# luuvish/arrow-h264

Hardware: AMD Instinct MI355X
Metric: macroblocks/s (decode reconstruct, post-entropy) 1080p P-frame; % HBM roofline (higher is better)
Workload: dtype u8

## Files before the change

### arrow-h264_amd/csrc/k_recon.hip

```cpp
#include "kernels.h"
#include "mb_inter_sp.h"

using namespace h264r;

#ifndef H264R_INTER_WAVES
#define H264R_INTER_WAVES 4
#endif
struct LdsRegs {
    const uint8_t* plane;
    uint2 refs, hdr;
};
DEV LdsRegs inter4_lds_load(const h264r_batch& b, int pic)
{
    const int t = threadIdx.x;
    const int nsl = min(b.slice_stride, INTER4_LDS_SLICES);
    const h264r_slice* sl = b.slices + (size_t)pic * b.slice_stride;
    LdsRegs r;
    r.plane = b.ref_planes[(size_t)pic * b.ref_planes_stride + min(t, 3 * H264R_MAX_SLOTS - 1)];
    const int ri = min(t, nsl * 4 - 1);
    r.refs = *reinterpret_cast<const uint2*>(&sl[ri >> 2].ref_slot[0][0] + 8 * (ri & 3));
    r.hdr = *reinterpret_cast<const uint2*>(&sl[min(t, nsl - 1)]);
    return r;
}
DEV void inter4_lds_store(const h264r_batch& b, const LdsRegs& r, Inter4Lds& S)
{
    const int t = threadIdx.x;
    const int nsl = min(b.slice_stride, INTER4_LDS_SLICES);
    if (t < 3 * H264R_MAX_SLOTS) S.planes[t] = r.plane;
    if (t < nsl * 4) *reinterpret_cast<uint2*>(&S.ref_slot[t >> 2][0][0] + 8 * (t & 3)) = r.refs;
    if (t < nsl) {
        S.hdr[t] = r.hdr;
        S.slice_type[t] = (uint8_t)(r.hdr.x & 255);
    }
}
DEV void inter4_lds(const h264r_batch& b, int pic, Inter4Lds& S) { inter4_lds_store(b, inter4_lds_load(b, pic), S); }

DEV bool inter4_groups(const Geom& g, int2 rows, int per, int& grp, int& gend)
{
    const int groups = (g.wmb * (rows.y - rows.x) + 15) / 16, gb = (groups + 7) / 8;
    const int band = blockIdx.x & 7;
    grp = band * gb + (blockIdx.x >> 3) * per;
    gend = min(min(grp + per, (band + 1) * gb), groups);
    return grp < gend;
}

extern "C" __global__ __launch_bounds__(256, H264R_INTER_WAVES) void k_inter4r(h264r_batch b, DbInfo* dbinfo, int2 rows,
                                                                               int* sp_flag, uint8_t* recon, int tag,
                                                                               int* zero, int nz, int* zero2, int nz2)
{
    {
        const int nt = (int)(gridDim.x * gridDim.y * blockDim.x);
        const int t = (int)((blockIdx.y * gridDim.x + blockIdx.x) * blockDim.x + threadIdx.x);
        for (int i = t; i < nz; i += nt) zero[i] = 0;
        for (int i = t; i < nz2; i += nt) zero2[i] = 0;
    }
    __shared__ Inter4Lds S;
    __shared__ DbTables T;
    const int pic = blockIdx.y;
    const Geom g = make_geom(b.width_mbs, b.height_mbs);
    int grp, gend;
    if (!inter4_groups(g, rows, H264R_INTER_GROUPS, grp, gend)) return;
    const int lane = threadIdx.x & 63, wave = __builtin_amdgcn_readfirstlane(threadIdx.x >> 6);
    const int aend = rows.y * g.wmb;
    const h264r_slice* slices = b.slices + (size_t)pic * b.slice_stride;
    int a0 = rows.x * g.wmb + (grp * 4 + wave) * 4;
    const uint2 tv = db_tables_load(threadIdx.x);
    Inter4Pre pre = inter4_pre(b, g, pic, a0, aend, lane);
    DbNb nb = dbinfo_pre(b, g, pic, a0, aend, lane);
    const LdsRegs lr = inter4_lds_load(b, pic);
    const int ns = (int)ld_const(&b.pics[pic].num_slices);
    db_tables_store(T, threadIdx.x, tv);
    inter4_lds_store(b, lr, S);
    inter4_plain_mark(S, threadIdx.x, lr.hdr, ns);
    __syncthreads();
    const bool plain = inter4_plain_picture(b, S, ns);
    for (;;) {
        if (a0 >= aend) return;
        bool done = false;
        if ((H264R_INTER_FAST & 2) && plain && inter4_plain_wave(pre, nb, ns)) {
            const uint2 m0 = motion_word<true>(pre.mv[0], pre.ri[0], slices, S, pre.q.slice, 0);
            done = (H264R_INTER_DIAG & 32) ||
                   dbinfo_block<true>(b, pic, inter4_lane(g, a0, aend, lane), S, T, pre.q, m0, inter4_no_list(),
                                      slice_hdr<true>(slices, S, pre.q.slice), nb, dbinfo + (size_t)pic * g.nmb, true);
            if (done) {
                int ln = lane;
                asm volatile("" : "+v"(ln));
                inter4_mbs<true>(b, g, pic, a0, aend, ln, S, sp_flag, pre, recon, tag);
            }
        }
        if (!done) {
            {
                const uint2 m0 = motion_word(pre.mv[0], pre.ri[0], slices, S, pre.q.slice, 0);
                const bool one = (H264R_INTER_FAST & 2) && inter4_one_list(pre, nb);
                uint2 m1 = inter4_no_list();
                if (!one) m1 = motion_word(pre.mv[1], pre.ri[1], slices, S, pre.q.slice, 1);
                if (!(H264R_INTER_DIAG & 32))
                    dbinfo_block(b, pic, inter4_lane(g, a0, aend, lane), S, T, pre.q, m0, m1,
                                 slice_hdr(slices, S, pre.q.slice), nb, dbinfo + (size_t)pic * g.nmb, one);
            }
            int ln = lane;
            asm volatile("" : "+v"(ln));
            inter4_mbs(b, g, pic, a0, aend, ln, S, sp_flag, pre, recon, tag);
        }
        if (++grp >= gend) return;
        a0 = rows.x * g.wmb + (grp * 4 + wave) * 4;
        int ln2 = lane;
        asm volatile("" : "+v"(ln2));
        pre = inter4_pre(b, g, pic, a0, aend, ln2);
        nb = dbinfo_pre(b, g, pic, a0, aend, ln2);
    }
}


extern "C" __global__ __launch_bounds__(256) void k_inter_sp(h264r_batch b, int2 rows, const int* sp_flag, uint8_t* recon,
                                                             int tag)
{
    if (__hip_atomic_load(sp_flag, __ATOMIC_RELAXED, __HIP_MEMORY_SCOPE_AGENT) != tag) return;
    __shared__ Inter4Lds S;
    const Geom g = make_geom(b.width_mbs, b.height_mbs);
    const int lane = threadIdx.x & 63, wave = __builtin_amdgcn_readfirstlane(threadIdx.x >> 6);
    const int groups = (g.wmb * (rows.y - rows.x) + 15) / 16;
    const int aend = rows.y * g.wmb;
    for (int w = blockIdx.x; w < groups * b.num_pics; w += gridDim.x) {
        const int pic = w / groups, grp = w % groups;
        __syncthreads();
        inter4_lds(b, pic, S);
        __syncthreads();
        const int a0 = rows.x * g.wmb + (grp * 4 + wave) * 4;
        if (a0 < aend) inter4_sp_mbs(b, g, pic, a0, aend, lane, S, recon);
    }
}

extern "C" __global__ __launch_bounds__(256) void k_untile(h264r_batch b, int2 rows, const uint8_t* __restrict__ recon)
{
    const Geom g = make_geom(b.width_mbs, b.height_mbs);
    const int pic = blockIdx.y;
    const int t = blockIdx.x * 256 + threadIdx.x, a = rows.x * g.wmb + (t >> 5), k = t & 31;
    if (a >= rows.y * g.wmb) return;
    const int mbx = a % g.wmb, mby = a / g.wmb;
    const uint8_t* mb = recon + ((size_t)pic * g.nmb + a) * RECON_MB;
    if (k < 16) {
        *reinterpret_cast<uint4*>(b.out_y + (size_t)pic * g.ysz + (size_t)(mby * 16 + k) * g.W + mbx * 16) =
            *reinterpret_cast<const uint4*>(mb + k * 16);
    } else {
        const int pl = (k - 16) >> 3, r = k & 7;
        uint8_t* dst = (pl ? b.out_v : b.out_u) + (size_t)pic * g.csz + (size_t)(mby * 8 + r) * g.Wc + mbx * 8;
        *reinterpret_cast<uint2*>(dst) = *reinterpret_cast<const uint2*>(mb + RECON_CB + pl * 64 + r * 8);
    }
}

extern "C" __global__ __launch_bounds__(256) void k_derive444(h264r_batch b, int pl, int qpl, h264r_mb* __restrict__ mbs,
                                                              h264r_slice* __restrict__ slices, h264r_quant* __restrict__ quant,
                                                              const uint8_t** __restrict__ refs, int ntab, int* err)
{
    const int64_t nt = (int64_t)gridDim.x * blockDim.x, t0 = (int64_t)blockIdx.x * blockDim.x + threadIdx.x;
    const int64_t nmb = (int64_t)b.width_mbs * b.height_mbs, P = b.num_pics;
    for (int64_t i = t0; i < P * nmb; i += nt) {
        h264r_mb m = b.mbs[i];
        const int cbpl = m.cbp & 15;
        if (m.mb_type == H264R_I_PCM) m.coef_off += 128u * (uint32_t)pl;
        else m.coef_off += (uint32_t)(pl * (64 * __builtin_popcount(cbpl) + (m.mb_type == H264R_I_16x16 ? 16 : 0)));
        if (pl) { m.qp_y = m.qp_c[pl - 1]; m.qp_scaled[0] = m.qp_scaled[pl]; }
        m.cbp = (uint8_t)cbpl;
        m.chroma_mode = 0;
        mbs[i] = m;
    }
    for (int64_t i = t0; i < P * b.slice_stride; i += nt) {
        h264r_slice x = b.slices[i];
        if (x.slice_type == H264R_SLICE_SP) atomicOr(err, DEV_ERR_FORMAT);
        if (pl) {
            for (int l = 0; l < 2; ++l)
                for (int r = 0; r < H264R_MAX_REFS; ++r) {
                    x.wp_weight[l][r][0] = x.wp_weight[l][r][pl];
                    x.wp_offset[l][r][0] = x.wp_offset[l][r][pl];
                }
            x.luma_log2_wd = x.chroma_log2_wd;
        }
        slices[i] = x;
    }
    constexpr int QW = (int)(sizeof(h264r_quant) / 2);
    constexpr int S4 = 3 * 6 * 16, S8 = 3 * 6 * 64;
    for (int64_t i = t0; i < P * QW; i += nt) {
        const int64_t q = i / QW;
        int k = (int)(i % QW);
        const int16_t* src = reinterpret_cast<const int16_t*>(b.quant + q);
        int from = k;
        if (k < 2 * S4) {
            const int half = k / S4, r = k % S4;
            if (r < 6 * 16) from = half * S4 + qpl * 6 * 16 + r;
        } else {
            const int k8 = k - 2 * S4, half = k8 / S8, r = k8 % S8;
            if (r < 6 * 64) from = 2 * S4 + half * S8 + qpl * 6 * 64 + r;
        }
        reinterpret_cast<int16_t*>(quant + q)[k] = src[from];
    }
    for (int64_t i = t0; i < (int64_t)ntab * 3 * H264R_MAX_SLOTS; i += nt) {
        const int64_t tab = i / (3 * H264R_MAX_SLOTS), e = i % (3 * H264R_MAX_SLOTS), slot = e / 3;
        refs[i] = b.ref_planes[tab * b.ref_planes_stride + 3 * slot + qpl];
    }
    for (int64_t i = t0; i < P; i += nt)
        if (b.pics[i].structure != H264R_FRAME) atomicOr(err, DEV_ERR_NOT_FRAME);
}
```

### arrow-h264_amd/csrc/mb_inter4.h

```cpp
#pragma once
#include "mb_deblock.h"

#ifndef H264R_INTER_DIAG
#define H264R_INTER_DIAG 0
#endif
#ifndef H264R_INTER_FAST
#define H264R_INTER_FAST 3
#endif

namespace h264r {

constexpr int INTER4_MBS = 16;
constexpr int INTER4_LDS_SLICES = 64;
constexpr int INTER4_PLAIN_SLICES = 8;
static_assert(INTER4_PLAIN_SLICES <= INTER4_LDS_SLICES, "a plain picture's slices are all in the LDS copy");

struct Inter4Lds {
    const uint8_t* planes[3 * H264R_MAX_SLOTS];
    uint2 hdr[INTER4_LDS_SLICES];
    int8_t ref_slot[INTER4_LDS_SLICES][2][H264R_MAX_REFS];
    uint8_t slice_type[INTER4_LDS_SLICES];
    uint8_t not_plain[INTER4_PLAIN_SLICES];
};

struct Inter4Lane {
    int blk, bx, by;
    int aa;
    bool valid;
    int mbx, mby;
    int X4, Y4;
    int b8;
    int cb, cr, cc;
    int yoff, coff;
};
DEV Inter4Lane inter4_lane(const Geom& g, int a0, int aend, int lane)
{
    Inter4Lane L;
    const int blk = lane & 15, bx = blk & 3, by = blk >> 2, a = a0 + (lane >> 4);
    L.blk = blk; L.bx = bx; L.by = by;
    L.valid = a < aend;
    L.aa = L.valid ? a : aend - 1;
    L.mbx = L.aa % g.wmb; L.mby = L.aa / g.wmb;
    L.X4 = L.mbx * 4 + bx; L.Y4 = L.mby * 4 + by;
    L.b8 = L.cb = (by >> 1) * 2 + (bx >> 1);
    L.cr = (by & 1) * 2; L.cc = (bx & 1) * 2;
    L.yoff = (by * 4) * 16 + bx * 4;
    L.coff = RECON_CB + (by * 2) * 8 + bx * 2;
    return L;
}

DEV int slice_byte(const h264r_slice* slices, int slice, int off)
{
    const __amdgpu_buffer_rsrc_t rs = __builtin_amdgcn_make_buffer_rsrc(const_cast<h264r_slice*>(slices + slice), 0,
                                                                        (int)sizeof(h264r_slice), 0x00020000);
    return __builtin_amdgcn_raw_buffer_load_b8(rs, off, 0, 0);
}
template <bool NEAR = false>
DEV int slice_type_of(const h264r_slice* slices, const Inter4Lds& S, int slice)
{
    int t = S.slice_type[min(slice, INTER4_LDS_SLICES - 1)];
    if constexpr (!NEAR)
        if (slice >= INTER4_LDS_SLICES) t = slice_byte(slices, slice, (int)offsetof(h264r_slice, slice_type));
    return t;
}

template <bool NEAR = false>
DEV uint2 slice_hdr(const h264r_slice* slices, const Inter4Lds& S, int slice)
{
    if (NEAR || slice < INTER4_LDS_SLICES) return S.hdr[NEAR ? min(slice, INTER4_LDS_SLICES - 1) : slice];
    return *reinterpret_cast<const uint2*>(&slices[slice]);
}

template <bool NEAR = false>
DEV uint2 motion_word(uint32_t mv, int ri, const h264r_slice* slices, const Inter4Lds& S, int slice, int l)
{
    const bool has = ri >= 0 && ri < H264R_MAX_REFS;
    const int ric = has ? ri : 0;
    int slot = S.ref_slot[min(slice, INTER4_LDS_SLICES - 1)][l][ric];
    if constexpr (!NEAR)
        if (slice >= INTER4_LDS_SLICES)
            slot = (int8_t)slice_byte(slices, slice, (int)offsetof(h264r_slice, ref_slot) + l * H264R_MAX_REFS + ric);
    slot = has ? slot : -1;
    return make_uint2(mv, (uint32_t)(uint8_t)ri | ((uint32_t)(uint8_t)slot << 8));
}
DEV uint2 block_motion(const h264r_batch& b, const h264r_slice* slices, const Inter4Lds& S, size_t at, int slice, int l)
{
    return motion_word(b.mv[at], b.ref_idx[at], slices, S, slice, l);
}

DEV h264r_mb mb_lane(const h264r_mb* p)
{
    const uint4* q = reinterpret_cast<const uint4*>(p);
    const uint4 w0 = q[0], w1 = q[1];
    h264r_mb m;
    uint32_t* w = reinterpret_cast<uint32_t*>(&m);
    w[0] = w0.x; w[1] = w0.y; w[2] = w0.z; w[3] = w0.w; w[4] = w1.x; w[5] = w1.y; w[6] = w1.z; w[7] = w1.w;
    return m;
}

struct Inter4Pre {
    h264r_mb q;
    uint32_t mv[2];
    int ri[2];
};
DEV Inter4Pre inter4_pre(const h264r_batch& b, const Geom& g, int pic, int a0, int aend, int lane)
{
    const Inter4Lane L = inter4_lane(g, a0, aend, lane);
    const int mi = L.Y4 * g.W4 + L.X4;
    const size_t mbase = (size_t)pic * 2 * g.motion_plane;
    Inter4Pre p;
    p.q = mb_lane(&b.mbs[(size_t)pic * g.nmb + L.aa]);
#pragma unroll
    for (int l = 0; l < 2; ++l) {
        p.mv[l] = b.mv[mbase + l * g.motion_plane + mi];
        p.ri[l] = b.ref_idx[mbase + l * g.motion_plane + mi];
    }
    return p;
}

struct DbNb {
    h264r_mb L, U;
    uint32_t lmv[2], umv[2];
    int lri[2], uri[2];
};
DEV DbNb dbinfo_pre(const h264r_batch& b, const Geom& g, int pic, int a0, int aend, int lane)
{
    const Inter4Lane L = inter4_lane(g, a0, aend, lane);
    const int aa = L.aa, mi = L.Y4 * g.W4 + L.X4;
    const int li = L.X4 > 0 ? mi - 1 : mi, ui = L.Y4 > 0 ? mi - g.W4 : mi;
    const size_t mbase = (size_t)pic * 2 * g.motion_plane;
    const h264r_mb* mbs = b.mbs + (size_t)pic * g.nmb;
    DbNb n;
    n.L = mb_lane(&mbs[L.mbx > 0 ? aa - 1 : aa]);
    n.U = mb_lane(&mbs[L.mby > 0 ? aa - g.wmb : aa]);
#pragma unroll
    for (int l = 0; l < 2; ++l) {
        n.lmv[l] = b.mv[mbase + l * g.motion_plane + li];
        n.lri[l] = b.ref_idx[mbase + l * g.motion_plane + li];
        n.umv[l] = b.mv[mbase + l * g.motion_plane + ui];
        n.uri[l] = b.ref_idx[mbase + l * g.motion_plane + ui];
    }
    return n;
}

DEV int sel16(uint32_t lo, uint32_t hi, int c) { return (int16_t)(((c & 2) ? hi : lo) >> (16 * (c & 1))); }

typedef short s16x2 __attribute__((ext_vector_type(2)));
typedef float f32x2 __attribute__((ext_vector_type(2)));
DEV s16x2 as_s16x2(uint32_t v) { return __builtin_bit_cast(s16x2, v); }
DEV uint32_t as_u32(s16x2 v) { return __builtin_bit_cast(uint32_t, v); }
DEV s16x2 splat16(short v) { return (s16x2){v, v}; }
DEV s16x2 pk_max(s16x2 a, s16x2 b) { return __builtin_elementwise_max(a, b); }
DEV s16x2 pk_min(s16x2 a, s16x2 b) { return __builtin_elementwise_min(a, b); }
DEV s16x2 pk_clip255(s16x2 a) { return pk_min(pk_max(a, splat16(0)), splat16(255)); }
DEV s16x2 pk_lo(uint32_t a, uint32_t b) { return as_s16x2(__builtin_amdgcn_perm(b, a, 0x05040100u)); }
DEV s16x2 pk_hi(uint32_t a, uint32_t b) { return as_s16x2(__builtin_amdgcn_perm(b, a, 0x07060302u)); }
DEV s16x2 pk_sat(int a, int b) { return __builtin_bit_cast(s16x2, __builtin_amdgcn_cvt_pk_i16(a, b)); }
DEV void idct4_pk(s16x2& a, s16x2& b, s16x2& c, s16x2& d)
{
    const s16x2 e0 = a + c, e1 = a - c, e2 = (b >> splat16(1)) - d, e3 = b + (d >> splat16(1));
    a = e0 + e3; b = e1 + e2; c = e1 - e2; d = e0 - e3;
}
constexpr uint32_t DQ4_BIAS = 1u << 27;
DEV uint32_t dq4_biased(int lev, int scale, int per) { return ((uint32_t)(lev * scale) * (1u << per) + 0x80000008u) >> 4; }
DEV uint32_t abs_acc_biased(uint32_t u, uint32_t acc)
{
    uint32_t r;
    asm("v_sad_u32 %0, %1, %2, %3" : "=v"(r) : "v"(u), "s"(DQ4_BIAS), "v"(acc));
    return r;
}
constexpr uint32_t PK_RES_MAX = 32700;
DEV uint32_t construct4(uint32_t pred, s16x2 r01, s16x2 r23)
{
    const s16x2 p01 = as_s16x2(__builtin_amdgcn_perm(0, pred, 0x0c010c00u)), p23 = as_s16x2(__builtin_amdgcn_perm(0, pred, 0x0c030c02u));
    const s16x2 s01 = pk_clip255(__builtin_elementwise_add_sat(p01, r01)), s23 = pk_clip255(__builtin_elementwise_add_sat(p23, r23));
    return __builtin_amdgcn_perm(as_u32(s23), as_u32(s01), 0x06040200u);
// ... 239 lines not shown
    const bool noref = !mb_is_intra(pre.q) && pre.ri[0] < 0;
    return inter4_one_list(pre, nb) && !__any(far || noref);
}

template <bool ONE>
DEV void dbinfo_records(const h264r_mb& q, const h264r_mb& L, const h264r_mb& U, const MotionRef& mq, const MotionRef& ml,
                        const MotionRef& mu, int blk, int hasL, int hasU, uint32_t qsh0, int l_type, int u_type, int fld,
                        const DbTables& T, DbInfo* __restrict__ out)
{
    const int bx = blk & 3, by = blk >> 2;
    const int q_type = qsh0 & 255, idc = (qsh0 >> 8) & 255;
    const int offa = (int8_t)((qsh0 >> 16) & 255), offb = (int8_t)(qsh0 >> 24);
    const int mvlim = fld ? 2 : 4;
    const int q_intra = mb_is_intra(q);
    const int fl = idc == 0 ? hasL : (idc == 2 && hasL && L.slice == q.slice);
    const int ft = idc == 0 ? hasU : (idc == 2 && hasU && U.slice == q.slice);
    const int t8 = (q.flags & H264R_MBF_T8x8) != 0;
    const int pskip = q_type == H264R_SLICE_P && q.mb_type == H264R_P_SKIP;
    const int special_q = special_slice(q_type);
#pragma unroll
    for (int hor = 0; hor < 2; ++hor) {
        const int e = hor ? by : bx, s = hor ? bx : by;
        const int en = idc != 1 && (e == 0 ? (hor ? ft : fl) : ((e & 1) ? !t8 : 1));
        int v = 0;
        if (en) {
            const int p_flags = e == 0 ? (hor ? U.flags : L.flags) : q.flags;
            const int p_cbp = e == 0 ? (hor ? U.cbp_blks : L.cbp_blks) : q.cbp_blks;
            const int special = special_q || (e == 0 && special_slice(hor ? u_type : l_type));
            const int intra = q_intra || (p_flags & H264R_MBF_INTRA) != 0;
            const int blkQ = 4 * by + bx;
            const int blkP = hor ? (e == 0 ? 12 + bx : blkQ - 4) : (e == 0 ? blkQ + 3 : blkQ - 1);
            const int coded = ((q.cbp_blks >> blkQ) & 1) || ((p_cbp >> blkP) & 1);
            const int same_part = e > 0 && (q.mb_type == H264R_P_16x16 ||
                                            q.mb_type == (hor ? H264R_P_8x16 : H264R_P_16x8));
            if (!hor) {
                if (special) v = e == 0 ? 4 : 3;
                else if (e > 0 && pskip) v = 0;
                else if (e == 0 && intra) v = 4;
                else if (intra) v = 3;
                else if (coded) v = 2;
                else if (same_part) v = 0;
                else v = ONE ? bs_compare_one(mq, ml, mvlim) : bs_compare(mq, ml, mvlim);
            } else {
                if (e == 0 && !fld && (special || intra)) v = 4;
                else if (special || intra) v = 3;
                else if (e > 0 && pskip) v = 0;
                else if (coded) v = 2;
                else if (same_part) v = 0;
                else v = ONE ? bs_compare_one(mq, mu, mvlim) : bs_compare(mq, mu, mvlim);
            }
        }
        out->bs[hor * 16 + e * 4 + s] = (uint8_t)v;
    }
    if (blk < 9) {
        const int pl = blk / 3, which = blk - pl * 3;
        const h264r_mb& P = which == 0 ? L : (which == 1 ? U : q);
        const int qp = mb_qp(P, pl), qq = mb_qp(q, pl);
        out->par[blk] = edge_word(qp, qq, offa, offb, T.ab, T.tc0);
    }
}

template <bool PLAIN = false>
DEV bool dbinfo_block(const h264r_batch& b, int pic, const Inter4Lane& ln, const Inter4Lds& S, const DbTables& T,
                      const h264r_mb& q, uint2 m0, uint2 m1, uint2 qsh, const DbNb& nb, DbInfo* __restrict__ dbout, bool one)
{
    const int bx = ln.bx, by = ln.by;
    const h264r_slice* slices = b.slices + (size_t)pic * b.slice_stride;
    const int hasL = ln.mbx > 0, hasU = ln.mby > 0;
    const h264r_mb& L = nb.L;
    const h264r_mb& U = nb.U;
    const int lsl = bx > 0 ? q.slice : L.slice, usl = by > 0 ? q.slice : U.slice;
    const uint2 l0 = motion_word<PLAIN>(nb.lmv[0], nb.lri[0], slices, S, lsl, 0);
    const uint2 u0 = motion_word<PLAIN>(nb.umv[0], nb.uri[0], slices, S, usl, 0);
    uint2 l1 = inter4_no_list(), u1 = l1;
    if constexpr (!PLAIN) {
        if (!one) {
            l1 = motion_word(nb.lmv[1], nb.lri[1], slices, S, lsl, 1);
            u1 = motion_word(nb.umv[1], nb.uri[1], slices, S, usl, 1);
        }
    }
    const int l_type = slice_type_of<PLAIN>(slices, S, L.slice), u_type = slice_type_of<PLAIN>(slices, S, U.slice);
    const int fld = (int)__builtin_amdgcn_readfirstlane(ld_const(&b.pics[pic].structure)) != H264R_FRAME;
    const MotionRef mq = motion_of(m0, m1), ml = motion_of(l0, l1), mu = motion_of(u0, u1);
    const bool both_missing = !mb_is_intra(q) && mq.ref[0] < 0 && (ml.ref[0] < 0 || mu.ref[0] < 0);
    if constexpr (PLAIN) {
        if (__any(ln.valid && both_missing)) return false;
    }
    if (ln.valid) {
        DbInfo* out = dbout + ln.aa;
        if constexpr (PLAIN) {
            dbinfo_records<true>(q, L, U, mq, ml, mu, ln.blk, hasL, hasU, qsh.x, l_type, u_type, fld, T, out);
        } else {
            if (one) one = !__any(both_missing);
            if (one) dbinfo_records<true>(q, L, U, mq, ml, mu, ln.blk, hasL, hasU, qsh.x, l_type, u_type, fld, T, out);
            else dbinfo_records<false>(q, L, U, mq, ml, mu, ln.blk, hasL, hasU, qsh.x, l_type, u_type, fld, T, out);
        }
    }
    return true;
}

DEV void inter4_pcm(uint8_t* rmb, const Inter4Lane& L, const int16_t* lv)
{
    const uint8_t* raw = reinterpret_cast<const uint8_t*>(lv);
#pragma unroll
    for (int r = 0; r < 4; ++r)
        *reinterpret_cast<uint32_t*>(rmb + L.yoff + r * 16) = *reinterpret_cast<const uint32_t*>(raw + (L.by * 4 + r) * 16 + L.bx * 4);
#pragma unroll
    for (int pl = 0; pl < 2; ++pl)
#pragma unroll
        for (int r = 0; r < 2; ++r)
            *reinterpret_cast<uint16_t*>(rmb + L.coff + pl * 64 + r * 8) =
                *reinterpret_cast<const uint16_t*>(raw + 256 + pl * 64 + (L.by * 2 + r) * 8 + L.bx * 2);
}

DEV void inter4_mc(const Geom& g, const Inter4Lane& L, const Inter4Lds& S, int structure, int fld, uint2 mw, int rr, bool use,
                   uint32_t (&tY)[4], uint32_t (&tC)[2])
{
    tY[0] = tY[1] = tY[2] = tY[3] = 0x80808080u;
    tC[0] = tC[1] = 0x80808080u;
    const int ref = (int8_t)((mw.y >> 8) & 255);
    const int slot = ref & 31, bot = fld & (ref >> 6);
    const bool ok = use && ref >= 0 && (ref & ~H264R_REF_BOTTOM) < H264R_MAX_SLOTS && rr < H264R_MAX_REFS &&
                    S.planes[slot * 3];
    const int mvx = (int16_t)(mw.x & 0xFFFF), mvy = (int16_t)(mw.x >> 16);
    const int vx = L.X4 * 16 + mvx, vy = L.Y4 * 16 + mvy;
    const int x = vx >> 2, y = vy >> 2;
    {
        uint32_t w[9][3];
        if constexpr (H264R_INTER_DIAG & 4) {
            tY[0] = tY[1] = tY[2] = tY[3] = (uint32_t)(vx ^ vy);
        } else {
            if (ok) luma_window_global(S.planes[slot * 3] + bot * g.W, g.W, g.W << fld, g.H, x, y, w);
            if constexpr (H264R_INTER_DIAG & 2) {
                if (ok) {
                    uint32_t acc = 0;
#pragma unroll
                    for (int r = 0; r < 9; ++r) acc ^= w[r][0] ^ w[r][1] ^ w[r][2];
                    tY[0] = tY[1] = tY[2] = tY[3] = acc;
                }
            } else {
                if (ok) luma_block_pred(w, g.W, x, vx & 3, vy & 3, tY);
            }
        }
    }
    const int vyc = vy + (fld && bot != (structure == H264R_BOTTOM_FIELD) ? (bot ? -2 : 2) : 0);
    if constexpr (H264R_INTER_DIAG & 8) {
        tC[0] = tC[1] = (uint32_t)vyc;
    } else {
        if (ok) chroma_block_pred2(S.planes[slot * 3 + 1] + bot * g.Wc, S.planes[slot * 3 + 2] + bot * g.Wc, g.Wc,
                                   g.Wc << fld, g.Hc, vx >> 3, vyc >> 3, vx & 7, vyc & 7, tC);
    }
}

template <bool PLAIN = false>
DEV void inter4_predict(const h264r_batch& b, const Geom& g, int pic, const Inter4Lane& L, const Inter4Lds& S,
                        const h264r_slice* __restrict__ qs, int wp_mode, uint2 m0, uint2 m1, uint32_t (&predY)[4],
                        uint32_t (&predC)[2])
{
    const int structure = (int)__builtin_amdgcn_readfirstlane(ld_const(&b.pics[pic].structure));
    const int fld = structure != H264R_FRAME;
    const int r0 = (int8_t)(m0.y & 255);
    if constexpr (PLAIN) {
        inter4_mc(g, L, S, structure, fld, m0, r0, true, predY, predC);
        return;
    }
    const int r1 = (int8_t)(m1.y & 255);
    const int dir = (r0 >= 0 && r1 >= 0) ? 2 : (r0 >= 0 ? 0 : 1);
    uint32_t pY[2][4] = {{0, 0, 0, 0}, {0, 0, 0, 0}}, pC[2][2] = {{0, 0}, {0, 0}};
#pragma unroll 1
    for (int l = 0; l < 2; ++l) {
        const uint2 mw = l ? m1 : m0;
        const int rr = l ? r1 : r0;
        const bool use = rr >= 0;
        if (!__any(use)) continue;
        uint32_t tY[4], tC[2];
        inter4_mc(g, L, S, structure, fld, mw, rr, use, tY, tC);
        const bool l1 = l != 0;
#pragma unroll
        for (int i = 0; i < 4; ++i) {
            pY[0][i] = (use && !l1) ? tY[i] : pY[0][i];
            pY[1][i] = (use && l1) ? tY[i] : pY[1][i];
        }
#pragma unroll
        for (int k = 0; k < 2; ++k) {
            pC[0][k] = (use && !l1) ? tC[k] : pC[0][k];
            pC[1][k] = (use && l1) ? tC[k] : pC[1][k];
        }
    }
    WpPar wpp[3] = {};
    if (wp_mode != 0) {
        const WpRaw wr = wp_raw(qs, r0, r1);
#pragma unroll
        for (int pl = 0; pl < 3; ++pl) wpp[pl] = wp_params(wr, wp_mode, dir, pl);
    }
#pragma unroll
    for (int i = 0; i < 4; ++i) predY[i] = wp_combine4(wpp[0], wp_mode, dir, pY[0][i], pY[1][i]);
#pragma unroll
    for (int pl = 0; pl < 2; ++pl) predC[pl] = wp_combine4(wpp[1 + pl], wp_mode, dir, pC[0][pl], pC[1][pl]);
}

struct Inter4Res {
    uint4 lev[2], lsc[2];
    uint32_t clev[2][2], csc[2][2];
    uint2 cdc[2];
    int cdcs[2];
};
DEV Inter4Res inter4_res_load(const h264r_mb& q, const Inter4Lane& L, const int16_t* lv, const h264r_quant* __restrict__ qt)
{
    Inter4Res R = {};
    const int cbpc = q.cbp >> 4, qpl = q.qp_scaled[0];
    const int by = L.by, bx = L.bx;
    const int loff = b8_offset(q.cbp, L.b8);
    if (loff >= 0) {
        if (!(q.flags & H264R_MBF_T8x8)) {
            const uint4* p = reinterpret_cast<const uint4*>(lv + loff + ((by & 1) * 2 + (bx & 1)) * 16);
            R.lev[0] = p[0]; R.lev[1] = p[1];
            const uint4* s = reinterpret_cast<const uint4*>(&qt->scale4x4[1][0][qpl % 6][0]);
            R.lsc[0] = s[0]; R.lsc[1] = s[1];
        } else {
            const int16_t* p = lv + loff + (by & 1) * 32 + (bx & 1) * 4;
            const int16_t* s = &qt->scale8x8[1][0][qpl % 6][(by & 1) * 32 + (bx & 1) * 4];
            const uint2 r0 = ld8(p), r1 = ld8(p + 8), r2 = ld8(p + 16), r3 = ld8(p + 24);
            R.lev[0] = make_uint4(r0.x, r0.y, r1.x, r1.y); R.lev[1] = make_uint4(r2.x, r2.y, r3.x, r3.y);
            const uint2 s0 = ld8(s), s1 = ld8(s + 8), s2 = ld8(s + 16), s3 = ld8(s + 24);
            R.lsc[0] = make_uint4(s0.x, s0.y, s1.x, s1.y); R.lsc[1] = make_uint4(s2.x, s2.y, s3.x, s3.y);
        }
    }
    if (cbpc) {
        const LevelOffs lo = level_offsets(q);
#pragma unroll
        for (int pl = 0; pl < 2; ++pl) {
            const int qpc = q.qp_scaled[1 + pl];
            R.cdc[pl] = ld8(lv + lo.cdc + pl * 4);
            R.cdcs[pl] = qt->scale4x4[1][1 + pl][qpc % 6][0];
            if (cbpc == 2) {
#pragma unroll
                for (int r = 0; r < 2; ++r) {
                    R.clev[pl][r] = *reinterpret_cast<const uint32_t*>(lv + lo.cac + pl * 64 + L.cb * 16 + (L.cr + r) * 4 + L.cc);
                    R.csc[pl][r] = *reinterpret_cast<const uint32_t*>(&qt->scale4x4[1][1 + pl][qpc % 6][(L.cr + r) * 4 + L.cc]);
                }
            }
        }
    }
    return R;
}
DEV int res_at(const uint4 (&w)[2], int i, int c) { return sel16((i & 1) ? w[i >> 1].z : w[i >> 1].x, (i & 1) ? w[i >> 1].w : w[i >> 1].y, c); }
DEV int level_at(const Inter4Res& R, int i, int c) { return res_at(R.lev, i, c); }
DEV int scale_at(const Inter4Res& R, int i, int c) { return res_at(R.lsc, i, c); }
DEV void luma_dequant(const Inter4Res& R, int per, int t8, int (&d)[4][4])
{
    const int drnd = t8 ? 32 : 8, dsh = t8 ? 6 : 4;
#pragma unroll
    for (int i = 0; i < 4; ++i)
#pragma unroll
        for (int c = 0; c < 4; ++c) d[i][c] = ((level_at(R, i, c) * scale_at(R, i, c)) * (1 << per) + drnd) >> dsh;
}
DEV void pack_res(const int (&res)[4][4], s16x2 (&rp)[4][2])
{
#pragma unroll
    for (int i = 0; i < 4; ++i) {
        rp[i][0] = pk_sat(res[i][0], res[i][1]);
        rp[i][1] = pk_sat(res[i][2], res[i][3]);
    }
}

DEV void luma_res_bypass(const h264r_mb& q, const Inter4Lane& L, const Inter4Res& R, int t8, s16x2 (&rp)[4][2])
{
    const int bx = L.bx, by = L.by;
    int d[4][4];
#pragma unroll
    for (int i = 0; i < 4; ++i)
#pragma unroll
        for (int c = 0; c < 4; ++c) d[i][c] = level_at(R, i, c);
    const uint32_t* qw = reinterpret_cast<const uint32_t*>(&q);
    const uint64_t ipw = (uint64_t)qw[5] | ((uint64_t)qw[6] << 32);
    const int bk = t8 ? L.b8 : (by >> 1) * 8 + (bx >> 1) * 4 + (by & 1) * 2 + (bx & 1);
    const int mode = (int)((ipw >> (4 * bk)) & 15);
    const bool vert = mode == 0, horz = mode == 1;
#pragma unroll
    for (int i = 1; i < 4; ++i)
#pragma unroll
        for (int c = 0; c < 4; ++c) d[i][c] += vert ? d[i - 1][c] : 0;
#pragma unroll
    for (int c = 1; c < 4; ++c)
#pragma unroll
        for (int i = 0; i < 4; ++i) d[i][c] += horz ? d[i][c - 1] : 0;
#pragma unroll
    for (int c = 0; c < 4; ++c) {
        const int up = lane_xor4(d[3][c]);
#pragma unroll
        for (int i = 0; i < 4; ++i) d[i][c] += (t8 && vert && (by & 1)) ? up : 0;
    }
#pragma unroll
    for (int i = 0; i < 4; ++i) {
        const int left = lane_xor1(d[i][3]);
#pragma unroll
        for (int c = 0; c < 4; ++c) d[i][c] += (t8 && horz && (bx & 1)) ? left : 0;
    }
    pack_res(d, rp);
}

template <bool PK>
DEV void luma_res_4x4(const Inter4Res& R, int per, int t8, s16x2 (&rp)[4][2])
{
    bool pk = PK;
    uint32_t u[4][4];
    if (pk) {
        uint32_t gs = 0;
#pragma unroll
        for (int i = 0; i < 4; ++i)
#pragma unroll
            for (int c = 0; c < 4; ++c) {
                u[i][c] = dq4_biased(level_at(R, i, c), scale_at(R, i, c), per);
                gs = abs_acc_biased(u[i][c], gs);
            }
        pk = !__any(gs > PK_RES_MAX);
    }
    if (pk) {
        s16x2 A[4], B[4];
#pragma unroll
        for (int c = 0; c < 4; ++c) {
            A[c] = pk_lo(u[0][c], u[1][c]);
            B[c] = pk_lo(u[2][c], u[3][c]);
        }
        A[0] += (s16x2){32, 0};
        idct4_pk(A[0], A[1], A[2], A[3]);
        idct4_pk(B[0], B[1], B[2], B[3]);
#pragma unroll
        for (int h = 0; h < 2; ++h) {
            s16x2 x0 = pk_lo(as_u32(A[2 * h]), as_u32(A[2 * h + 1])), x1 = pk_hi(as_u32(A[2 * h]), as_u32(A[2 * h + 1]));
            s16x2 x2 = pk_lo(as_u32(B[2 * h]), as_u32(B[2 * h + 1])), x3 = pk_hi(as_u32(B[2 * h]), as_u32(B[2 * h + 1]));
            idct4_pk(x0, x1, x2, x3);
            rp[0][h] = x0 >> splat16(6); rp[1][h] = x1 >> splat16(6);
            rp[2][h] = x2 >> splat16(6); rp[3][h] = x3 >> splat16(6);
        }
    } else {
        int d[4][4], res[4][4];
        if constexpr (PK) {
#pragma unroll
            for (int i = 0; i < 4; ++i)
#pragma unroll
                for (int c = 0; c < 4; ++c) d[i][c] = (int)(u[i][c] - DQ4_BIAS);
        } else {
            luma_dequant(R, per, t8, d);
        }
        idct4x4_inplace(d);
#pragma unroll
        for (int i = 0; i < 4; ++i)
#pragma unroll
            for (int c = 0; c < 4; ++c) res[i][c] = (d[i][c] + 32) >> 6;
        pack_res(res, rp);
    }
}

DEV void luma_res_8x8(const Inter4Lane& L, const Inter4Res& R, int per, int t8, s16x2 (&rp)[4][2])
{
    const int bx = L.bx, by = L.by;
    int d[4][4], e4[4][4], res[4][4];
    luma_dequant(R, per, t8, d);
#pragma unroll
    for (int i = 0; i < 4; ++i) {
        int in[8], outv[8];
#pragma unroll
        for (int c = 0; c < 4; ++c) {
            const int ov = lane_xor1(d[i][c]);
            in[c] = (bx & 1) ? ov : d[i][c];
            in[4 + c] = (bx & 1) ? d[i][c] : ov;
        }
        idct8(in, outv);
        const int mx = -(bx & 1);
#pragma unroll
        for (int c = 0; c < 4; ++c) e4[i][c] = (outv[c] & ~mx) | (outv[4 + c] & mx);
    }
#pragma unroll
    for (int c = 0; c < 4; ++c) {
        int in[8], outv[8];
#pragma unroll
        for (int i = 0; i < 4; ++i) {
            in[i] = lane_lo4(e4[i][c]);
            in[4 + i] = lane_hi4(e4[i][c]);
        }
        idct8(in, outv);
        const int my = -(by & 1);
#pragma unroll
        for (int i = 0; i < 4; ++i) res[i][c] = t8 ? ((outv[i] & ~my) | (outv[4 + i] & my)) : 0;
    }
    if (!t8) idct4x4_inplace(d);
#pragma unroll
    for (int i = 0; i < 4; ++i)
#pragma unroll
        for (int c = 0; c < 4; ++c) res[i][c] = ((t8 ? res[i][c] : d[i][c]) + 32) >> 6;
    pack_res(res, rp);
}

template <bool PK>
DEV void inter4_luma_residual(const h264r_mb& q, const Inter4Lane& L, const Inter4Res& R, s16x2 (&rp)[4][2])
{
#pragma unroll
    for (int i = 0; i < 4; ++i) rp[i][0] = rp[i][1] = splat16(0);
    if (!__any((q.cbp & 15) != 0)) return;
    const int t8 = (q.flags & H264R_MBF_T8x8) != 0, per = q.qp_scaled[0] / 6;
    if (q.flags & H264R_MBF_BYPASS) luma_res_bypass(q, L, R, t8, rp);
    else if (!__any(t8 != 0)) luma_res_4x4<PK>(R, per, t8, rp);
    else luma_res_8x8(L, R, per, t8, rp);
}
DEV void luma_res_stub(const Inter4Res& R, s16x2 (&rp)[4][2])
{
#pragma unroll
    for (int i = 0; i < 4; ++i) rp[i][0] = rp[i][1] = splat16(0);
    rp[0][0].x = (short)((R.lev[0].x ^ R.lev[0].y ^ R.lev[0].z ^ R.lev[0].w ^ R.lev[1].x ^ R.lev[1].y ^ R.lev[1].z ^ R.lev[1].w ^
                          R.lsc[0].x ^ R.lsc[1].y) & 3);
}

DEV void inter4_store_luma(uint8_t* rmb, const Inter4Lane& L, const uint32_t (&predY)[4], const s16x2 (&rp)[4][2])
{
#pragma unroll
    for (int i = 0; i < 4; ++i) *reinterpret_cast<uint32_t*>(rmb + L.yoff + i * 16) = construct4(predY[i], rp[i][0], rp[i][1]);
}
DEV void inter4_store_luma_16b(uint8_t* rmb, const Inter4Lane& L, const uint32_t (&predY)[4], const s16x2 (&rp)[4][2])
{
    uint32_t wv4[4];
#pragma unroll
    for (int i = 0; i < 4; ++i) wv4[i] = construct4(predY[i], rp[i][0], rp[i][1]);
    *reinterpret_cast<uint4*>(rmb + L.blk * 16) = make_uint4(wv4[0], wv4[1], wv4[2], wv4[3]);
}

DEV s16x2 lane_xor1(s16x2 v) { return as_s16x2((uint32_t)lane_xor1((int)as_u32(v))); }
DEV s16x2 lane_lo4(s16x2 v) { return as_s16x2((uint32_t)lane_lo4((int)as_u32(v))); }
DEV s16x2 lane_hi4(s16x2 v) { return as_s16x2((uint32_t)lane_hi4((int)as_u32(v))); }
template <auto Op, typename T>
DEV void quad_rows(T& a, T& b, int cc)
{
    const T o0 = lane_xor1(a), o1 = lane_xor1(b);
    T d0 = cc ? o0 : a, d1 = cc ? o1 : b, d2 = cc ? a : o0, d3 = cc ? b : o1;
    Op(d0, d1, d2, d3);
    a = cc ? d2 : d0;
    b = cc ? d3 : d1;
}
template <auto Op, bool XOR4 = false, typename T>
DEV void quad_cols(T& a, T& b, int cr)
{
    T d0, d1, d2, d3;
    if constexpr (XOR4) {
        const T o0 = lane_xor4(a), o1 = lane_xor4(b);
        d0 = cr ? o0 : a; d1 = cr ? o1 : b; d2 = cr ? a : o0; d3 = cr ? b : o1;
    } else {
        d0 = lane_lo4(a); d1 = lane_lo4(b); d2 = lane_hi4(a); d3 = lane_hi4(b);
    }
    Op(d0, d1, d2, d3);
    a = cr ? d2 : d0;
    b = cr ? d3 : d1;
}

template <bool PK>
DEV void inter4_chroma_residual(const h264r_mb& q, const Inter4Lane& L, const Inter4Res& R, s16x2 (&rcp)[2][2])
{
    const int cb = L.cb, cr = L.cr, cc = L.cc;
    const int cbpc = q.cbp >> 4;
    const bool byp = (q.flags & H264R_MBF_BYPASS) != 0;
#pragma unroll
    for (int pl = 0; pl < 2; ++pl) rcp[pl][0] = rcp[pl][1] = splat16(0);
    if (!__any(cbpc != 0)) return;
    const bool dcl_lane = cr == 0 && cc == 0;
    uint32_t k[2][2][2];
    int dcl[2];
#pragma unroll
    for (int pl = 0; pl < 2; ++pl) {
        const int qpc = q.qp_scaled[1 + pl], per = qpc / 6;
#pragma unroll
        for (int r = 0; r < 2; ++r)
#pragma unroll
            for (int c = 0; c < 2; ++c)
                k[pl][r][c] = dq4_biased((int16_t)(R.clev[pl][r] >> (16 * c)), (int16_t)(R.csc[pl][r] >> (16 * c)), per);
        const int c00 = (int16_t)(R.cdc[pl].x & 0xFFFF), c01 = (int16_t)(R.cdc[pl].x >> 16);
        const int c10 = (int16_t)(R.cdc[pl].y & 0xFFFF), c11 = (int16_t)(R.cdc[pl].y >> 16);
        const int e00 = c00 + c01, e01 = c00 - c01, e10 = c10 + c11, e11 = c10 - c11;
        const int ea = (cb & 1) ? e01 : e00, eb = (cb & 1) ? e11 : e10;
        const int f = ea + (eb ^ -(cb >> 1)) + (cb >> 1);
        if (dcl_lane) k[pl][0][0] = (uint32_t)(cbpc ? ((f * R.cdcs[pl]) * (1 << per)) >> 5 : 0) + DQ4_BIAS;
        dcl[pl] = cb == 0 ? c00 : cb == 1 ? c01 : cb == 2 ? c10 : c11;
    }
    bool pk = PK;
    if (pk) {
        uint32_t gs[2];
#pragma unroll
        for (int pl = 0; pl < 2; ++pl)
            gs[pl] = abs_acc_biased(k[pl][0][0], abs_acc_biased(k[pl][0][1], abs_acc_biased(k[pl][1][0], abs_acc_biased(k[pl][1][1], 0))));
        int m = byp ? 0 : (int)max(gs[0], gs[1]);
        int o = lane_xor1(m);
        asm volatile("" : "+v"(o));
        m = (int)((uint32_t)m + (uint32_t)o);
        int lo = lane_lo4(m), hi = lane_hi4(m);
        asm volatile("" : "+v"(lo), "+v"(hi));
        pk = !__any((uint32_t)lo + (uint32_t)hi > PK_RES_MAX);
    }
    if (pk) {
        s16x2 K[2][2];
#pragma unroll
        for (int r = 0; r < 2; ++r)
#pragma unroll
            for (int c = 0; c < 2; ++c) K[r][c] = pk_lo(k[0][r][c], k[1][r][c]);
        K[0][0] += splat16(dcl_lane ? 32 : 0);
#pragma unroll
        for (int r = 0; r < 2; ++r) quad_rows<idct4_pk>(K[r][0], K[r][1], cc);
#pragma unroll
        for (int c = 0; c < 2; ++c) quad_cols<idct4_pk>(K[0][c], K[1][c], cr);
#pragma unroll
        for (int r = 0; r < 2; ++r) {
            const uint32_t r0 = as_u32(K[r][0] >> splat16(6)), r1 = as_u32(K[r][1] >> splat16(6));
            rcp[0][r] = pk_lo(r0, r1);
            rcp[1][r] = pk_hi(r0, r1);
        }
    } else {
#pragma unroll
        for (int pl = 0; pl < 2; ++pl) {
            int t[2][2];
#pragma unroll
            for (int r = 0; r < 2; ++r) {
                t[r][0] = (int)(k[pl][r][0] - DQ4_BIAS);
                t[r][1] = (int)(k[pl][r][1] - DQ4_BIAS);
                quad_rows<idct4_inplace>(t[r][0], t[r][1], cc);
            }
#pragma unroll
            for (int c = 0; c < 2; ++c) quad_cols<idct4_inplace>(t[0][c], t[1][c], cr);
#pragma unroll
            for (int r = 0; r < 2; ++r) rcp[pl][r] = pk_sat((t[r][0] + 32) >> 6, (t[r][1] + 32) >> 6);
        }
    }
    if (byp) {
#pragma unroll
        for (int pl = 0; pl < 2; ++pl) {
            rcp[pl][0] = dcl_lane ? pk_hi((uint32_t)dcl[pl] << 16, R.clev[pl][0]) : as_s16x2(R.clev[pl][0]);
            rcp[pl][1] = as_s16x2(R.clev[pl][1]);
        }
    }
}
DEV void chroma_res_stub(const Inter4Res& R, s16x2 (&rcp)[2][2])
{
#pragma unroll
    for (int pl = 0; pl < 2; ++pl) {
        rcp[pl][0] = rcp[pl][1] = splat16(0);
        rcp[pl][0].x = (short)((R.clev[pl][0] ^ R.clev[pl][1] ^ R.csc[pl][0] ^ R.csc[pl][1] ^ R.cdc[pl].x ^ R.cdc[pl].y ^ (uint32_t)R.cdcs[pl]) & 3);
    }
}

DEV void inter4_store_chroma(uint8_t* rmb, const Inter4Lane& L, const uint32_t (&predC)[2], const s16x2 (&rcp)[2][2])
{
#pragma unroll
    for (int pl = 0; pl < 2; ++pl) {
        uint8_t* cdst = rmb + L.coff + pl * 64;
#pragma unroll
        for (int r = 0; r < 2; ++r) {
            const s16x2 pr = as_s16x2(__builtin_amdgcn_perm(0, predC[pl], r ? 0x0c030c02u : 0x0c010c00u));
            const s16x2 sv = pk_clip255(__builtin_elementwise_add_sat(pr, rcp[pl][r]));
            *reinterpret_cast<uint16_t*>(cdst + r * 8) = (uint16_t)__builtin_amdgcn_perm(0, as_u32(sv), 0x0c0c0200u);
        }
    }
}

template <bool PLAIN = false>
DEV void inter4_mbs(const h264r_batch& b, const Geom& g, int pic, int a0, int aend, int lane,
                    const Inter4Lds& S, int* sp_flag, const Inter4Pre& pre, uint8_t* __restrict__ recon, int tag)
{
    constexpr int DIAG = H264R_INTER_DIAG;
    constexpr bool PK = (H264R_INTER_FAST & 1) != 0;
    const Inter4Lane L = inter4_lane(g, a0, aend, lane);
    const h264r_slice* slices = b.slices + (size_t)pic * b.slice_stride;
    const h264r_mb q = pre.q;
    const uint2 qsh = slice_hdr<PLAIN>(slices, S, q.slice);
    const uint2 m0 = motion_word<PLAIN>(pre.mv[0], pre.ri[0], slices, S, q.slice, 0);
    uint2 m1 = inter4_no_list();
    if constexpr (!PLAIN) m1 = motion_word(pre.mv[1], pre.ri[1], slices, S, q.slice, 1);

    const bool pcm = q.mb_type == H264R_I_PCM;
    if (!L.valid || (mb_is_intra(q) && !pcm)) return;
    if constexpr (!PLAIN)
        if ((qsh.x & 255) == H264R_SLICE_SP && !mb_is_intra(q)) { *sp_flag = tag; return; }
    if (pcm) { inter4_pcm(recon_mb(recon, g, pic, L.aa), L, b.levels + q.coef_off); return; }

    uint32_t predY[4], predC[2];
    inter4_predict<PLAIN>(b, g, pic, L, S, &slices[q.slice], qsh.y & 255, m0, m1, predY, predC);
    Inter4Res R = {};
    if constexpr (!(DIAG & 16)) R = inter4_res_load(q, L, b.levels + q.coef_off, &b.quant[pic]);
    uint8_t* const rmb = recon_mb(recon, g, pic, L.aa);

    s16x2 rp[4][2];
    if constexpr (DIAG & (16 | 64)) luma_res_stub(R, rp);
    else inter4_luma_residual<PK>(q, L, R, rp);
    if constexpr (DIAG & 1) inter4_store_luma_16b(rmb, L, predY, rp);
    else inter4_store_luma(rmb, L, predY, rp);

    s16x2 rcp[2][2];
    if constexpr (DIAG & (16 | 128)) chroma_res_stub(R, rcp);
    else inter4_chroma_residual<PK>(q, L, R, rcp);
    inter4_store_chroma(rmb, L, predC, rcp);
}

}
```

Before: 745.3 million.

## Park live prediction and MB state in LDS to raise wave occupancy

Adds a per-thread LDS parking area where the non-plain inter path spills prediction words, list-1 motion, and selected macroblock record fields across the residual decode, then reloads them. It also raises the occupancy target in launch bounds from 4 to 5 waves. The bypass residual now reads its intra-mode dwords straight from global memory instead of keeping them live. The aim is lower VGPR pressure so more waves fit per SIMD. The cost is about 18KB of extra LDS per block plus extra LDS traffic, and the LDS growth may itself cap occupancy.

```diff
diff --git a/arrow-h264_amd/csrc/k_recon.hip b/arrow-h264_amd/csrc/k_recon.hip
--- a/arrow-h264_amd/csrc/k_recon.hip
+++ b/arrow-h264_amd/csrc/k_recon.hip
@@ -4,7 +4,7 @@
 using namespace h264r;
 
 #ifndef H264R_INTER_WAVES
-#define H264R_INTER_WAVES 4
+#define H264R_INTER_WAVES 5
 #endif
 struct LdsRegs {
     const uint8_t* plane;
@@ -56,6 +56,7 @@
     }
     __shared__ Inter4Lds S;
     __shared__ DbTables T;
+    __shared__ Inter4Park P;
     const int pic = blockIdx.y;
     const Geom g = make_geom(b.width_mbs, b.height_mbs);
     int grp, gend;
@@ -78,14 +79,16 @@
         if (a0 >= aend) return;
         bool done = false;
         if ((H264R_INTER_FAST & 2) && plain && inter4_plain_wave(pre, nb, ns)) {
-            const uint2 m0 = motion_word<true>(pre.mv[0], pre.ri[0], slices, S, pre.q.slice, 0);
+            uint2 m0 = motion_word<true>(pre.mv[0], pre.ri[0], slices, S, pre.q.slice, 0);
+            asm volatile("" : "+v"(m0.y));
             done = (H264R_INTER_DIAG & 32) ||
                    dbinfo_block<true>(b, pic, inter4_lane(g, a0, aend, lane), S, T, pre.q, m0, inter4_no_list(),
                                       slice_hdr<true>(slices, S, pre.q.slice), nb, dbinfo + (size_t)pic * g.nmb, true);
             if (done) {
                 int ln = lane;
-                asm volatile("" : "+v"(ln));
-                inter4_mbs<true>(b, g, pic, a0, aend, ln, S, sp_flag, pre, recon, tag);
+                uint2 mm = m0;
+                asm volatile("" : "+v"(ln), "+v"(mm.x), "+v"(mm.y));
+                inter4_mbs<true>(b, g, pic, a0, aend, ln, S, sp_flag, pre, recon, tag, nullptr, mm);
             }
         }
         if (!done) {
@@ -100,7 +103,7 @@
             }
             int ln = lane;
             asm volatile("" : "+v"(ln));
-            inter4_mbs(b, g, pic, a0, aend, ln, S, sp_flag, pre, recon, tag);
+            inter4_mbs(b, g, pic, a0, aend, ln, S, sp_flag, pre, recon, tag, &P);
         }
         if (++grp >= gend) return;
         a0 = rows.x * g.wmb + (grp * 4 + wave) * 4;
diff --git a/arrow-h264_amd/csrc/mb_inter4.h b/arrow-h264_amd/csrc/mb_inter4.h
--- a/arrow-h264_amd/csrc/mb_inter4.h
+++ b/arrow-h264_amd/csrc/mb_inter4.h
@@ -22,6 +22,34 @@
     uint8_t slice_type[INTER4_LDS_SLICES];
     uint8_t not_plain[INTER4_PLAIN_SLICES];
 };
+
+constexpr int PARK_PRED = 0;
+constexpr int PARK_M1 = 12;
+constexpr int PARK_Q = 14;
+constexpr int INTER4_PARK_SLOTS = 18;
+struct Inter4Park {
+    uint32_t w[INTER4_PARK_SLOTS][256];
+};
+typedef __attribute__((address_space(3))) volatile uint32_t lds_vdword;
+DEV void park_put(Inter4Park& P, int slot, uint32_t v) { *(lds_vdword*)&P.w[slot][threadIdx.x] = v; }
+DEV uint32_t park_get(Inter4Park& P, int slot) { return *(lds_vdword*)&P.w[slot][threadIdx.x]; }
+constexpr int PARK_Q_N = 4;
+constexpr int PARK_Q_WORD[PARK_Q_N] = {0, 3, 2, 4};
+DEV void park_put_mb(Inter4Park& P, const h264r_mb& q)
+{
+    const uint32_t* w = reinterpret_cast<const uint32_t*>(&q);
+#pragma unroll
+    for (int k = 0; k < PARK_Q_N; ++k) park_put(P, PARK_Q + k, w[PARK_Q_WORD[k]]);
+}
+template <int FIRST = PARK_Q_N>
+DEV h264r_mb park_get_mb(Inter4Park& P)
+{
+    h264r_mb q = {};
+    uint32_t* w = reinterpret_cast<uint32_t*>(&q);
+#pragma unroll
+    for (int k = 0; k < FIRST; ++k) w[PARK_Q_WORD[k]] = park_get(P, PARK_Q + k);
+    return q;
+}
 
 struct Inter4Lane {
     int blk, bx, by;
@@ -567,10 +595,10 @@
     }
 }
 
-template <bool PLAIN = false>
+template <bool PLAIN = false, bool PARK = false>
 DEV void inter4_predict(const h264r_batch& b, const Geom& g, int pic, const Inter4Lane& L, const Inter4Lds& S,
                         const h264r_slice* __restrict__ qs, int wp_mode, uint2 m0, uint2 m1, uint32_t (&predY)[4],
-                        uint32_t (&predC)[2])
+                        uint32_t (&predC)[2], Inter4Park* park = nullptr)
 {
     const int structure = (int)__builtin_amdgcn_readfirstlane(ld_const(&b.pics[pic].structure));
     const int fld = structure != H264R_FRAME;
@@ -581,29 +609,56 @@
     }
     const int r1 = (int8_t)(m1.y & 255);
     const int dir = (r0 >= 0 && r1 >= 0) ? 2 : (r0 >= 0 ? 0 : 1);
+    if constexpr (PARK) {
+        park_put(*park, PARK_M1, m1.x);
+        park_put(*park, PARK_M1 + 1, m1.y);
+    }
     uint32_t pY[2][4] = {{0, 0, 0, 0}, {0, 0, 0, 0}}, pC[2][2] = {{0, 0}, {0, 0}};
+    bool parked[2] = {false, false};
 #pragma unroll 1
     for (int l = 0; l < 2; ++l) {
-        const uint2 mw = l ? m1 : m0;
         const int rr = l ? r1 : r0;
         const bool use = rr >= 0;
         if (!__any(use)) continue;
+        uint2 mw = l ? m1 : m0;
+        if constexpr (PARK)
+            if (l) mw = make_uint2(park_get(*park, PARK_M1), park_get(*park, PARK_M1 + 1));
         uint32_t tY[4], tC[2];
         inter4_mc(g, L, S, structure, fld, mw, rr, use, tY, tC);
         const bool l1 = l != 0;
-#pragma unroll
-        for (int i = 0; i < 4; ++i) {
-            pY[0][i] = (use && !l1) ? tY[i] : pY[0][i];
-            pY[1][i] = (use && l1) ? tY[i] : pY[1][i];
-        }
-#pragma unroll
-        for (int k = 0; k < 2; ++k) {
-            pC[0][k] = (use && !l1) ? tC[k] : pC[0][k];
-            pC[1][k] = (use && l1) ? tC[k] : pC[1][k];
-        }
+        if constexpr (PARK) {
+#pragma unroll
+            for (int i = 0; i < 4; ++i) park_put(*park, PARK_PRED + 6 * l + i, use ? tY[i] : 0);
+#pragma unroll
+            for (int k = 0; k < 2; ++k) park_put(*park, PARK_PRED + 6 * l + 4 + k, use ? tC[k] : 0);
+            parked[0] |= !l1;
+            parked[1] |= l1;
+        } else {
+#pragma unroll
+            for (int i = 0; i < 4; ++i) {
+                pY[0][i] = (use && !l1) ? tY[i] : pY[0][i];
+                pY[1][i] = (use && l1) ? tY[i] : pY[1][i];
+            }
+#pragma unroll
+            for (int k = 0; k < 2; ++k) {
+                pC[0][k] = (use && !l1) ? tC[k] : pC[0][k];
+                pC[1][k] = (use && l1) ? tC[k] : pC[1][k];
+            }
+        }
+    }
+    if constexpr (PARK) {
+#pragma unroll
+        for (int l = 0; l < 2; ++l)
+            if (parked[l]) {
+#pragma unroll
+                for (int i = 0; i < 4; ++i) pY[l][i] = park_get(*park, PARK_PRED + 6 * l + i);
+#pragma unroll
+                for (int k = 0; k < 2; ++k) pC[l][k] = park_get(*park, PARK_PRED + 6 * l + 4 + k);
+            }
     }
     WpPar wpp[3] = {};
     if (wp_mode != 0) {
+        if constexpr (PARK) qs += park_get(*park, PARK_Q + 2) >> 16;
         const WpRaw wr = wp_raw(qs, r0, r1);
 #pragma unroll
         for (int pl = 0; pl < 3; ++pl) wpp[pl] = wp_params(wr, wp_mode, dir, pl);
@@ -679,7 +734,7 @@
     }
 }
 
-DEV void luma_res_bypass(const h264r_mb& q, const Inter4Lane& L, const Inter4Res& R, int t8, s16x2 (&rp)[4][2])
+DEV void luma_res_bypass(const h264r_mb* __restrict__ qg, const Inter4Lane& L, const Inter4Res& R, int t8, s16x2 (&rp)[4][2])
 {
     const int bx = L.bx, by = L.by;
     int d[4][4];
@@ -687,7 +742,8 @@
     for (int i = 0; i < 4; ++i)
 #pragma unroll
         for (int c = 0; c < 4; ++c) d[i][c] = level_at(R, i, c);
-    const uint32_t* qw = reinterpret_cast<const uint32_t*>(&q);
+    const uint32_t* qw = reinterpret_cast<const uint32_t*>(qg);
+    static_assert(offsetof(h264r_mb, ipred) == 20, "dwords 5 and 6 of the record");
     const uint64_t ipw = (uint64_t)qw[5] | ((uint64_t)qw[6] << 32);
     const int bk = t8 ? L.b8 : (by >> 1) * 8 + (bx >> 1) * 4 + (by & 1) * 2 + (bx & 1);
     const int mode = (int)((ipw >> (4 * bk)) & 15);
@@ -808,16 +864,27 @@
     pack_res(res, rp);
 }
 
-template <bool PK>
-DEV void inter4_luma_residual(const h264r_mb& q, const Inter4Lane& L, const Inter4Res& R, s16x2 (&rp)[4][2])
+template <bool PK, bool PARK = false>
+DEV void inter4_luma_residual(const h264r_mb& q, const h264r_mb* __restrict__ qg, const Inter4Lane& L, const Inter4Res& R,
+                              s16x2 (&rp)[4][2], uint32_t (&predY)[4], Inter4Park* park = nullptr)
 {
 #pragma unroll
     for (int i = 0; i < 4; ++i) rp[i][0] = rp[i][1] = splat16(0);
     if (!__any((q.cbp & 15) != 0)) return;
     const int t8 = (q.flags & H264R_MBF_T8x8) != 0, per = q.qp_scaled[0] / 6;
-    if (q.flags & H264R_MBF_BYPASS) luma_res_bypass(q, L, R, t8, rp);
+    if (q.flags & H264R_MBF_BYPASS) luma_res_bypass(qg, L, R, t8, rp);
     else if (!__any(t8 != 0)) luma_res_4x4<PK>(R, per, t8, rp);
-    else luma_res_8x8(L, R, per, t8, rp);
+    else {
+        if constexpr (PARK) {
+#pragma unroll
+            for (int i = 0; i < 4; ++i) park_put(*park, PARK_PRED + i, predY[i]);
+        }
+        luma_res_8x8(L, R, per, t8, rp);
+        if constexpr (PARK) {
+#pragma unroll
+            for (int i = 0; i < 4; ++i) predY[i] = park_get(*park, PARK_PRED + i);
+        }
+    }
 }
 DEV void luma_res_stub(const Inter4Res& R, s16x2 (&rp)[4][2])
 {
@@ -975,40 +1042,61 @@
 
 template <bool PLAIN = false>
 DEV void inter4_mbs(const h264r_batch& b, const Geom& g, int pic, int a0, int aend, int lane,
-                    const Inter4Lds& S, int* sp_flag, const Inter4Pre& pre, uint8_t* __restrict__ recon, int tag)
+                    const Inter4Lds& S, int* sp_flag, const Inter4Pre& pre, uint8_t* __restrict__ recon, int tag,
+                    Inter4Park* park = nullptr, uint2 m0_plain = make_uint2(0, 0))
 {
     constexpr int DIAG = H264R_INTER_DIAG;
     constexpr bool PK = (H264R_INTER_FAST & 1) != 0;
     const Inter4Lane L = inter4_lane(g, a0, aend, lane);
     const h264r_slice* slices = b.slices + (size_t)pic * b.slice_stride;
-    const h264r_mb q = pre.q;
-    const uint2 qsh = slice_hdr<PLAIN>(slices, S, q.slice);
-    const uint2 m0 = motion_word<PLAIN>(pre.mv[0], pre.ri[0], slices, S, q.slice, 0);
+    const h264r_mb q0 = pre.q;
+    const uint2 qsh = slice_hdr<PLAIN>(slices, S, q0.slice);
+    const uint2 m0 = PLAIN ? m0_plain : motion_word<PLAIN>(pre.mv[0], pre.ri[0], slices, S, q0.slice, 0);
     uint2 m1 = inter4_no_list();
-    if constexpr (!PLAIN) m1 = motion_word(pre.mv[1], pre.ri[1], slices, S, q.slice, 1);
-
-    const bool pcm = q.mb_type == H264R_I_PCM;
-    if (!L.valid || (mb_is_intra(q) && !pcm)) return;
+    if constexpr (!PLAIN) m1 = motion_word(pre.mv[1], pre.ri[1], slices, S, q0.slice, 1);
+
+    const bool pcm = q0.mb_type == H264R_I_PCM;
+    if (!L.valid || (mb_is_intra(q0) && !pcm)) return;
     if constexpr (!PLAIN)
-        if ((qsh.x & 255) == H264R_SLICE_SP && !mb_is_intra(q)) { *sp_flag = tag; return; }
-    if (pcm) { inter4_pcm(recon_mb(recon, g, pic, L.aa), L, b.levels + q.coef_off); return; }
+        if ((qsh.x & 255) == H264R_SLICE_SP && !mb_is_intra(q0)) { *sp_flag = tag; return; }
+    if (pcm) { inter4_pcm(recon_mb(recon, g, pic, L.aa), L, b.levels + q0.coef_off); return; }
 
     uint32_t predY[4], predC[2];
-    inter4_predict<PLAIN>(b, g, pic, L, S, &slices[q.slice], qsh.y & 255, m0, m1, predY, predC);
+    if constexpr (PLAIN) {
+        inter4_predict<true>(b, g, pic, L, S, &slices[q0.slice], qsh.y & 255, m0, m1, predY, predC);
+    } else {
+        park_put_mb(*park, q0);
+        inter4_predict<false, true>(b, g, pic, L, S, slices, qsh.y & 255, m0, m1, predY, predC, park);
+    }
+    h264r_mb q = q0;
+    Inter4Lane Lr = L;
+    if constexpr (!PLAIN) {
+        q = park_get_mb(*park);
+        int ln = lane;
+        asm volatile("" : "+v"(ln));
+        Lr = inter4_lane(g, a0, aend, ln);
+#pragma unroll
+        for (int pl = 0; pl < 2; ++pl) park_put(*park, PARK_PRED + 4 + pl, predC[pl]);
+    }
     Inter4Res R = {};
-    if constexpr (!(DIAG & 16)) R = inter4_res_load(q, L, b.levels + q.coef_off, &b.quant[pic]);
-    uint8_t* const rmb = recon_mb(recon, g, pic, L.aa);
+    if constexpr (!(DIAG & 16)) R = inter4_res_load(q, Lr, b.levels + q.coef_off, &b.quant[pic]);
+    uint8_t* const rmb = recon_mb(recon, g, pic, Lr.aa);
 
     s16x2 rp[4][2];
     if constexpr (DIAG & (16 | 64)) luma_res_stub(R, rp);
-    else inter4_luma_residual<PK>(q, L, R, rp);
-    if constexpr (DIAG & 1) inter4_store_luma_16b(rmb, L, predY, rp);
-    else inter4_store_luma(rmb, L, predY, rp);
-
+    else inter4_luma_residual<PK, !PLAIN>(q, &b.mbs[(size_t)pic * g.nmb + Lr.aa], Lr, R, rp, predY, park);
+    if constexpr (DIAG & 1) inter4_store_luma_16b(rmb, Lr, predY, rp);
+    else inter4_store_luma(rmb, Lr, predY, rp);
+
+    if constexpr (!PLAIN) {
+#pragma unroll
+        for (int pl = 0; pl < 2; ++pl) predC[pl] = park_get(*park, PARK_PRED + 4 + pl);
+        q = park_get_mb<2>(*park);
+    }
     s16x2 rcp[2][2];
     if constexpr (DIAG & (16 | 128)) chroma_res_stub(R, rcp);
-    else inter4_chroma_residual<PK>(q, L, R, rcp);
-    inter4_store_chroma(rmb, L, predC, rcp);
-}
-
-}
+    else inter4_chroma_residual<PK>(q, Lr, R, rcp);
+    inter4_store_chroma(rmb, Lr, predC, rcp);
+}
+
+}
```

After: 767.2 million, median of 6. +2.9%, better.
